# citiususc/veryfasttree

Hardware: AMD Instinct MI355X
Metric: profile-ops/sec (higher is better)
Workload: dtype f32; 1 GPU; c4_1M_x200_nt_tophits; n_seqs=1000000, n_pos=200, active_nodes=750000, top_k=2000

## Files before the change

veryfasttree_amd/csrc/vft_kernels_nj.h:

```cpp
#pragma once
#include "vft_device.h"

#define VFT_WG 256

template <typename REAL>
struct QueryBuf {
    REAL *w;
    uint8_t *code;
    REAL *f;
    uint4 *enc;
    double2 *tab;
};

template <typename REAL>
__device__ __forceinline__ void vft_query_tab(const QueryBuf<REAL> &q, int64_t p, REAL wq, const REAL *f) {
#pragma unroll
    for (int c = 0; c < 5; c++) {
        double2 v = make_double2(0.0, 0.0);
        if (c < 4 && wq > 0) {
            const double wgt = (double) wq;
            const double piece = 1.0 - (double) f[c < 4 ? c : 0];
            v = make_double2(wgt * piece, wgt);
        }
        q.tab[p * 5 + c] = v;
    }
}

template <typename REAL, int NC>
__device__ __forceinline__ void vft_extract_query(const Arena<REAL> &A, int64_t node, const QueryBuf<REAL> &q) {
    const int64_t p = (int64_t) blockIdx.x * blockDim.x + threadIdx.x;
    const int64_t nPosPad = (int64_t) A.d.nChunk * VFT_CHUNK;
    if (p >= nPosPad) return;
    REAL w = 0;
    int code = VFT_NOCODE_;
    REAL f[NC];
#pragma unroll
    for (int k = 0; k < NC; k++) f[k] = 0;
    if (p < A.d.nPos) {
        Col<REAL, NC> c;
        vft_load_col<REAL, NC>(A, node, p, c);
        w = c.w;
        code = c.code;
        if (c.vec) {
#pragma unroll
            for (int k = 0; k < NC; k++) f[k] = c.f[k];
        } else if (NC == 4 && code != VFT_NOCODE_) {
#pragma unroll
            for (int k = 0; k < NC; k++) f[k] = (k == code) ? (REAL) 1 : (REAL) 0;
        }
    }
    q.w[p] = w;
    q.code[p] = (uint8_t) code;
#pragma unroll
    for (int k = 0; k < NC; k++) q.f[p * NC + k] = f[k];
    if (NC == 4) vft_query_tab<REAL>(q, p, w, f);
    if (node < A.d.nSeqs && p < A.d.nChunk) {
        q.enc[p] = A.leafT[vft_leaf_idx(A.d, node >> 6, (int) p, (int) (node & 63))];
    }
}
template <typename REAL, int NC>
__global__ void k_extract_query(Arena<REAL> A, int64_t node, QueryBuf<REAL> q) {
    vft_extract_query<REAL, NC>(A, node, q);
}
#ifdef VFT_NO_PLAIN_COLUMNS
#define VFT_PLAIN_COLUMNS 0
#define VFT_MQ_STRIDE(S) (4 * (S) + 4)
#else
#define VFT_PLAIN_COLUMNS 1
#define VFT_MQ_STRIDE(S) (4 * (S) + 8)
#endif
#ifdef VFT_NO_SEED_CODE_RECORDS
#define VFT_SEED_CODE_RECORDS 0
#else
#define VFT_SEED_CODE_RECORDS 1
#endif
#if defined(VFT_NO_GPR_INDEX_SELECT) || !VFT_SEED_CODE_RECORDS || !VFT_PLAIN_COLUMNS
#define VFT_GPR_INDEX_SELECT 0
#else
#define VFT_GPR_INDEX_SELECT 1
#endif
template <typename REAL>
struct QuerySlot {
    int64_t node;
    QueryBuf<REAL> q;
    REAL *mq;
    int32_t mqIdx, mqS;
    uint32_t *lq;
    int32_t lqIdx, lqS;
};
template <typename REAL, int NC>
__global__ void k_extract_query_batch(Arena<REAL> A, const QuerySlot<REAL> *qs) {
    const QuerySlot<REAL> &sl = qs[blockIdx.y];
    vft_extract_query<REAL, NC>(A, sl.node, sl.q);
    if (VFT_SEED_CODE_RECORDS && NC == 4 && sl.lq) {
        const int64_t p = (int64_t) blockIdx.x * blockDim.x + threadIdx.x;
        if (p < (int64_t) A.d.nChunk * VFT_CHUNK) {
            uint8_t *dst = (uint8_t *) (sl.lq + p);
            dst[sl.lqIdx] = sl.q.code[p];
            if (sl.lqIdx == 0)
                for (int k = sl.lqS; k < 4; k++) dst[k] = VFT_NOCODE_;
        }
    }
    if (NC == 4 && sl.mq) {
        const int64_t p = (int64_t) blockIdx.x * blockDim.x + threadIdx.x;
        if (p < (int64_t) A.d.nChunk * VFT_CHUNK) {
            REAL *dst = sl.mq + p * VFT_MQ_STRIDE(sl.mqS);
#pragma unroll
            for (int k = 0; k < 4; k++) dst[4 * sl.mqIdx + k] = sl.q.f[p * 4 + k];
            dst[4 * sl.mqS + sl.mqIdx] = sl.q.w[p];
            if (VFT_PLAIN_COLUMNS) ((uint8_t *) (dst + 4 * sl.mqS + 4))[sl.mqIdx] = sl.q.code[p];
        }
    }
}

template <typename REAL, int NC>
__global__ void k_outprofile_as_query(Arena<REAL> A, QueryBuf<REAL> q) {
    const int64_t p = (int64_t) blockIdx.x * blockDim.x + threadIdx.x;
    const int64_t nPosPad = (int64_t) A.d.nChunk * VFT_CHUNK;
    if (p >= nPosPad) return;
    const bool in = p < A.d.nPos;
    q.w[p] = in ? A.outW[p] : (REAL) 0;
    q.code[p] = VFT_NOCODE_;
    REAL f[NC];
#pragma unroll
    for (int k = 0; k < NC; k++) {
        f[k] = in ? A.outF[p * NC + k] : (REAL) 0;
        q.f[p * NC + k] = f[k];
    }
    if (NC == 4) vft_query_tab<REAL>(q, p, in ? A.outW[p] : (REAL) 0, f);
}

struct SweepArgs {
    int64_t query;
    int64_t lo, hi;
    int64_t nActive, nDiffAllow;
    double totdiam;
    int32_t queryIsLeaf;
    int32_t force;
    int32_t nLeafWG;
    int32_t pad;
    int64_t leafEnd;
    int64_t heavyLo;
};

template <typename REAL>
struct SweepOut {
    REAL *dist, *weight, *crit;
    REAL *partMin, *partMax;
};

template <typename REAL, int NWAVES>
__device__ __forceinline__ void vft_block_minmax_n(REAL cmin, REAL cmax, REAL *partMin, REAL *partMax, int part) {
    __shared__ REAL smin[NWAVES], smax[NWAVES];
#pragma unroll
    for (int off = 32; off > 0; off >>= 1) {
        const REAL a = __shfl_xor(cmin, off, 64), b = __shfl_xor(cmax, off, 64);
        cmin = a < cmin ? a : cmin;
        cmax = b > cmax ? b : cmax;
    }
    if ((threadIdx.x & 63) == 0) {
        smin[threadIdx.x >> 6] = cmin;
        smax[threadIdx.x >> 6] = cmax;
    }
    __syncthreads();
    if (threadIdx.x == 0) {
#pragma unroll
        for (int w = 1; w < NWAVES; w++) {
            cmin = smin[w] < cmin ? smin[w] : cmin;
            cmax = smax[w] > cmax ? smax[w] : cmax;
        }
        partMin[part] = cmin;
        partMax[part] = cmax;
    }
}
template <typename REAL>
__device__ __forceinline__ void vft_block_minmax(REAL cmin, REAL cmax, REAL *partMin, REAL *partMax, int part) {
    vft_block_minmax_n<REAL, VFT_WG / 64>(cmin, cmax, partMin, partMax, part);
}

enum { MODE_CRIT = 0, MODE_OUTDIST = 1, MODE_CRIT_LEAFQ = 2 };

__device__ __forceinline__ void vft_seq_counts(const uint4 a, const uint4 b, int &nUse, int &nSame) {
    const uint32_t x = a.x & b.x, y = a.y & b.y, z = a.z & b.z, w = a.w & b.w;
    nUse += __popc(x & 0x10101010u) + __popc(y & 0x10101010u) + __popc(z & 0x10101010u) + __popc(w & 0x10101010u);
    nSame += __popc(x & 0x0F0F0F0Fu) + __popc(y & 0x0F0F0F0Fu) + __popc(z & 0x0F0F0F0Fu) + __popc(w & 0x0F0F0F0Fu);
}

#ifndef VFT_SUB
#define VFT_SUB 8
#endif
__device__ __forceinline__ uint32_t vft_query_code(const uint8_t *code, int64_t p0, int b) {
    const uint32_t w = vft_uniform_load<uint32_t>((const uint32_t *) (code + p0 + (b & ~3)));
    return (w >> ((b & 3) * 8)) & 0xFFu;
}
template <typename REAL>
__device__ __forceinline__ uint32_t vft_query_code(const QueryBuf<REAL> &Q, int64_t p0, int b) {
    return vft_query_code(Q.code, p0, b);
}

template <typename REAL, bool QLEAF>
struct IntChunk {
    REAL w[VFT_SUB];
    REAL f[VFT_SUB][QLEAF ? 1 : 4];
};

typedef unsigned int __attribute__((ext_vector_type(4))) vft_u4_t;
typedef unsigned int __attribute__((ext_vector_type(2))) vft_u2_t;
typedef const __attribute__((address_space(4))) vft_u4_t *vft_smask_t;
typedef const __attribute__((address_space(4))) vft_u2_t *vft_soff_t;

#ifdef VFT_ABLATE
#define VFT_ABLATE_BITS(s) ((s).pad)
#else
#define VFT_ABLATE_BITS(s) 0
#endif

template <typename REAL, bool QLEAF>
__device__ __forceinline__ void vft_int_chunk_load(IntChunk<REAL, QLEAF> &r, int c, int sub, const uint4 codes,
                                                   const REAL *wT, vft_smask_t mM, vft_soff_t mO, const REAL *fT,
                                                   const QueryBuf<REAL> &Q, int dbg = 0) {
    const int64_t p0 = (int64_t) c * VFT_CHUNK + sub * VFT_SUB;
    vft_u4_t mk[VFT_SUB];
    vft_u2_t of[VFT_SUB];
#pragma unroll
    for (int b = 0; b < VFT_SUB; b++) {
        mk[b] = mM[p0 + b];
        of[b] = mO[p0 + b];
    }
#pragma unroll
    for (int b = 0; b < VFT_SUB; b++) {
        const unsigned long long mv = ((unsigned long long) mk[b].y << 32) | mk[b].x;
        const unsigned long long mw = ((unsigned long long) mk[b].w << 32) | mk[b].z;
// ... 561 lines not shown
        cur = nxt;
    }
#endif
}

template <typename REAL, int S>
__global__ __launch_bounds__(VFT_WG) void k_sweep_nt_leafq_multi(Arena<REAL> A, MultiLeafQ<REAL, S> M, SweepArgs s) {
    constexpr int SUB = 8;
    REAL cmin[S], cmax[S];
#pragma unroll
    for (int q = 0; q < S; q++) {
        cmin[q] = (REAL) 1e30;
        cmax[q] = (REAL) -1e30;
    }
    const int wg = (int) gridDim.x - 1 - (int) blockIdx.x;
    const int64_t j = s.heavyLo + (int64_t) wg * VFT_WG + threadIdx.x;
    const int lane = (int) (j & 63);
    const int64_t tile = j >> 6;
    bool work = false;
    if (j < s.hi) {
        work = A.parent[j] < 0;
        if (!work) {
#pragma unroll
            for (int q = 0; q < S; q++) {
                M.O[q].dist[j] = (REAL) 1e20;
                M.O[q].crit[j] = (REAL) 1e20;
                M.O[q].weight[j] = 0;
            }
        }
    }
    if (work) {
        const bool targetLeaf = j < A.d.nSeqs;
        REAL dist[S], weight[S];
        if (targetLeaf) {
            int nUse[S], nSame[S];
#pragma unroll
            for (int q = 0; q < S; q++) nUse[q] = nSame[q] = 0;
            for (int c = 0; c < A.d.nChunk; c++) {
                const uint4 t = A.leafT[vft_leaf_idx(A.d, tile, c, lane)];
#pragma unroll
                for (int q = 0; q < S; q++) vft_seq_counts(t, M.Q[q].enc[c], nUse[q], nSame[q]);
            }
#pragma unroll
            for (int q = 0; q < S; q++) {
                const double top = (double) (nUse[q] - nSame[q]);
                weight[q] = (REAL) (double) nUse[q];
                dist[q] = (REAL) (nUse[q] > 0 ? top / (double) nUse[q] : 1.0);
            }
        } else {
            double top[S], denom[S];
#pragma unroll
            for (int q = 0; q < S; q++) top[q] = denom[q] = 0;
            LeafCodes<S> lc;
#if VFT_SEED_CODE_RECORDS
            lc.lq = M.lq;
#else
#pragma unroll
            for (int q = 0; q < S; q++) lc.code[q] = M.Q[q].code;
#endif
            vft_for_column_groups<REAL, SUB>(A, tile, lane, [&](const IntChunkAll<REAL, SUB> &ca, int64_t p0) {
                vft_int_chunk_consume_all<REAL, S, SUB>(ca, p0, lc, top, denom);
            });
#pragma unroll
            for (int q = 0; q < S; q++) {
                weight[q] = (REAL) (denom[q] > 0 ? denom[q] : 0.01);
                dist[q] = (REAL) (denom[q] > 0 ? top[q] / denom[q] : 1.0);
            }
        }
#pragma unroll
        for (int q = 0; q < S; q++) {
            SweepArgs sq = s;
            sq.query = M.query[q];
            vft_sweep_finish<REAL, MODE_CRIT>(A, sq, M.O[q], j, dist[q], weight[q], targetLeaf, cmin[q], cmax[q]);
        }
    }
    vft_block_minmax_multi<REAL, S>(cmin, cmax, M.O, wg);
}

template <int S>
__device__ __forceinline__ void vft_pin_sums(double *top, double *denom) {
#pragma unroll
    for (int q = 0; q < S; q++) asm volatile("" : "+v"(top[q]), "+v"(denom[q]));
}

template <typename REAL, int S>
struct QueryCol {
    REAL w[S];
    typename UVec4<REAL>::type f[S];
    uint32_t codes;
};
template <typename REAL, int S>
__device__ __forceinline__ void vft_query_col_load(QueryCol<REAL, S> &c, const REAL *mq, int64_t p) {
    const REAL *src = mq + p * VFT_MQ_STRIDE(S);
    const typename UVec4<REAL>::type wv = vft_uniform_load4<REAL>(src + 4 * S);
    if (VFT_PLAIN_COLUMNS) c.codes = vft_uniform_load<uint32_t>((const uint32_t *) (src + 4 * S + 4));
#pragma unroll
    for (int q = 0; q < S; q++) {
        c.w[q] = q == 0 ? wv.x : q == 1 ? wv.y : q == 2 ? wv.z : wv.w;
        c.f[q] = vft_uniform_load4<REAL>(src + 4 * q);
    }
}

template <typename REAL, int S, int SUB, bool ISEL = false>
__device__ __forceinline__ void vft_int_chunk_consume_prof(const IntChunkAll<REAL, SUB> &ca, int64_t p0, const REAL *mq, double *top, double *denom) {
    QueryCol<REAL, S> cur, nxt;
    vft_query_col_load<REAL, S>(cur, mq, p0);
#pragma unroll
    for (int b = 0; b < SUB; b++) {
        if (b + 1 < SUB) vft_query_col_load<REAL, S>(nxt, mq, p0 + b + 1);
        __builtin_amdgcn_sched_barrier(0);
#if VFT_SEED_CODE_RECORDS
        const unsigned long long cw = VFT_PLAIN_COLUMNS ? cur.codes : 0;
#endif
        constexpr bool isel = VFT_GPR_INDEX_SELECT && ISEL;
        double fd[S];
#if VFT_GPR_INDEX_SELECT
        if constexpr (ISEL) vft_isel_cvt<S>(fd, ca.f[b], b, cur.codes);
#endif
#pragma unroll
        for (int q = 0; q < S; q++) {
            const REAL ww = cur.w[q] * ca.w[b];
            const double wgt = (double) ww;
            double head = 1.0, lastd = 0;
            REAL last;
            if constexpr (isel) {
                lastd = fd[q];
            } else if (VFT_PLAIN_COLUMNS) {
#if VFT_SEED_CODE_RECORDS
                last = vft_usel_code(ca.f[b], cw, 8 * q);
#else
                const unsigned long long m0 = (cur.codes & (1u << (8 * q))) ? ~0ull : 0ull, m1 = (cur.codes & (2u << (8 * q))) ? ~0ull : 0ull;
                last = vft_usel(vft_usel(ca.f[b].x, ca.f[b].y, m0), vft_usel(ca.f[b].z, ca.f[b].w, m0), m1);
#endif
            }
            if (!VFT_PLAIN_COLUMNS || __builtin_expect((cur.codes & (0x40u << (8 * q))) != 0, 0)) {
                const typename UVec4<REAL>::type pr = cur.f[q] * ca.f[b];
                head = 1.0 - (double) pr.x;
                head -= (double) pr.y;
                head -= (double) pr.z;
                last = pr.w;
                if constexpr (isel) lastd = (double) pr.w;
            }
            if constexpr (!isel) lastd = (double) last;
            const double piece = head - lastd;
            denom[q] += wgt;
            top[q] += wgt * piece;
            if (VFT_PLAIN_COLUMNS) asm volatile("" : "+v"(top[q]), "+v"(denom[q]));
        }
        __builtin_amdgcn_sched_barrier(0);
        if (b + 1 < SUB) cur = nxt;
    }
}

#define VFT_PTILE_M 112
template <int NBT, int S>
__device__ __forceinline__ void vft_leaf_table_chunk_multi(const double2 *row, const uint4 *t, double (*top)[S], double (*denom)[S]) {
    constexpr int GC = NBT * S >= 8 ? 1 : NBT * S >= 4 ? 2 : 4;
#pragma unroll
    for (int g = 0; g < VFT_CHUNK; g += GC) {
        double2 v[NBT][GC][S];
#pragma unroll
        for (int bt = 0; bt < NBT; bt++)
#pragma unroll
            for (int q = 0; q < GC; q++) {
                const int idx = __ffs((int) (vft_byte(t[bt], g + q) | 0x10u)) - 1;
#pragma unroll
                for (int sd = 0; sd < S; sd++) v[bt][q][sd] = row[sd * (VFT_PTILE_M * 5) + (g + q) * 5 + idx];
            }
#pragma unroll
        for (int q = 0; q < GC; q++)
#pragma unroll
            for (int bt = 0; bt < NBT; bt++)
#pragma unroll
                for (int sd = 0; sd < S; sd++) {
                    denom[bt][sd] += v[bt][q][sd].y;
                    top[bt][sd] += v[bt][q][sd].x;
                }
    }
}

template <typename REAL, int NBT, int S>
__device__ __forceinline__ void vft_leaf_table_walk_multi(const Arena<REAL> &A, const MultiLeafQ<REAL, S> &M, double2 *tab, const int64_t *tj,
                                                          double (*top)[S], double (*denom)[S]) {
    const int tid = threadIdx.x;
    const int64_t nPos = A.d.nPos;
    const uint4 *lp[NBT];
#pragma unroll
    for (int bt = 0; bt < NBT; bt++) lp[bt] = A.leafT + vft_leaf_idx(A.d, tj[bt] >> 6, 0, (int) (tj[bt] & 63));
    for (int64_t p0 = 0; p0 < nPos; p0 += VFT_PTILE_M) {
        __syncthreads();
        {
            const int64_t nTab = ((int64_t) A.d.nChunk * VFT_CHUNK - p0) * 5;
#pragma unroll
            for (int sd = 0; sd < S; sd++)
                for (int e = tid; e < VFT_PTILE_M * 5; e += VFT_WG)
                    tab[sd * (VFT_PTILE_M * 5) + e] = e < nTab ? M.Q[sd].tab[p0 * 5 + e] : make_double2(0.0, 0.0);
        }
        __syncthreads();
        const int c0 = (int) (p0 / VFT_CHUNK);
        const int c1 = (int) (((p0 + VFT_PTILE_M < nPos ? p0 + VFT_PTILE_M : nPos) + VFT_CHUNK - 1) / VFT_CHUNK);
        uint4 ta[NBT], tb[NBT];
#pragma unroll
        for (int bt = 0; bt < NBT; bt++) ta[bt] = lp[bt][(int64_t) c0 * VFT_TILE];
        for (int c = c0; c < c1; c += 2) {
            const int cb = c + 1 < c1 ? c + 1 : c, ca = c + 2 < c1 ? c + 2 : c;
#pragma unroll
            for (int bt = 0; bt < NBT; bt++) tb[bt] = lp[bt][(int64_t) cb * VFT_TILE];
            __builtin_amdgcn_sched_barrier(0);
            vft_leaf_table_chunk_multi<NBT, S>(tab + (int64_t) (c - c0) * VFT_CHUNK * 5, ta, top, denom);
#pragma unroll
            for (int bt = 0; bt < NBT; bt++) ta[bt] = lp[bt][(int64_t) ca * VFT_TILE];
            __builtin_amdgcn_sched_barrier(0);
            if (c + 1 < c1) vft_leaf_table_chunk_multi<NBT, S>(tab + (int64_t) (c + 1 - c0) * VFT_CHUNK * 5, tb, top, denom);
        }
    }
}

template <typename REAL, int S>
__device__ __forceinline__ void vft_leaf_table_wg_multi(const Arena<REAL> &A, const MultiLeafQ<REAL, S> &M, const SweepArgs &s, int64_t base,
                                                        REAL *cmin, REAL *cmax) {
    constexpr int NB = VFT_LEAF_SPAN / VFT_WG, NW = VFT_WG / 64, NBT = 2;
    __shared__ double2 tab[S * VFT_PTILE_M * 5];
    __shared__ unsigned short list[VFT_LEAF_SPAN];
    __shared__ int segCnt[NB * NW];
    const int tid = threadIdx.x, wave = tid >> 6;
    unsigned long long bal[NB];
#pragma unroll
    for (int r = 0; r < NB; r++) {
        const int64_t j = base + r * VFT_WG + tid;
        bool active = false;
        if (j < s.leafEnd) {
            active = A.parent[j] < 0;
            if (!active) {
#pragma unroll
                for (int q = 0; q < S; q++) {
                    M.O[q].dist[j] = (REAL) 1e20;
                    M.O[q].crit[j] = (REAL) 1e20;
                    M.O[q].weight[j] = 0;
                }
            }
        }
        bal[r] = __ballot(active);
        if ((tid & 63) == 0) segCnt[r * NW + wave] = __popcll(bal[r]);
    }
    __syncthreads();
    int nAct = 0, off[NB];
#pragma unroll
    for (int seg = 0; seg < NB * NW; seg++) {
#pragma unroll
        for (int r = 0; r < NB; r++)
            if (seg == r * NW + wave) off[r] = nAct;
        nAct += segCnt[seg];
    }
#pragma unroll
    for (int r = 0; r < NB; r++) {
        const int rank = (int) __builtin_amdgcn_mbcnt_hi((unsigned int) (bal[r] >> 32), __builtin_amdgcn_mbcnt_lo((unsigned int) bal[r], 0u));
        if ((bal[r] >> (tid & 63)) & 1ull) list[off[r] + rank] = (unsigned short) (r * VFT_WG + tid);
    }
    __syncthreads();
    for (int r0 = 0; r0 < nAct; r0 += NBT * VFT_WG) {
        int64_t tj[NBT];
        double top[NBT][S], denom[NBT][S];
#pragma unroll
        for (int bt = 0; bt < NBT; bt++) {
            const int idx = r0 + bt * VFT_WG + tid;
            tj[bt] = base + list[idx < nAct ? idx : 0];
#pragma unroll
            for (int q = 0; q < S; q++) top[bt][q] = denom[bt][q] = 0;
        }
        if (nAct - r0 <= VFT_WG) vft_leaf_table_walk_multi<REAL, 1, S>(A, M, tab, tj, top, denom);
        else vft_leaf_table_walk_multi<REAL, NBT, S>(A, M, tab, tj, top, denom);
#pragma unroll
        for (int bt = 0; bt < NBT; bt++) {
            if (r0 + bt * VFT_WG + tid < nAct) {
#pragma unroll
                for (int q = 0; q < S; q++) {
                    const REAL weight = (REAL) (denom[bt][q] > 0 ? denom[bt][q] : 0.01);
                    const REAL dist = (REAL) (denom[bt][q] > 0 ? top[bt][q] / denom[bt][q] : 1.0);
                    SweepArgs sq = s;
                    sq.query = M.query[q];
                    vft_sweep_finish<REAL, MODE_CRIT>(A, sq, M.O[q], tj[bt], dist, weight, false, cmin[q], cmax[q]);
                }
            }
        }
    }
}

#define VFT_KARG __attribute__((address_space(4)))
template <typename T>
__device__ __forceinline__ const VFT_KARG T *vft_kernarg(size_t off) {
    const VFT_KARG char *p = (const VFT_KARG char *) __builtin_amdgcn_kernarg_segment_ptr() + off;
    asm volatile("" : "+s"(p));
    return (const VFT_KARG T *) p;
}
template <typename REAL>
__device__ __forceinline__ SweepOut<REAL> vft_karg_out(const VFT_KARG SweepOut<REAL> *p) {
    typedef __attribute__((address_space(1))) REAL *gp_t;
    SweepOut<REAL> o;
    o.dist = (REAL *) (gp_t) p->dist;
    o.weight = (REAL *) (gp_t) p->weight;
    o.crit = (REAL *) (gp_t) p->crit;
    o.partMin = (REAL *) (gp_t) p->partMin;
    o.partMax = (REAL *) (gp_t) p->partMax;
    return o;
}
template <typename REAL, int S>
__device__ __forceinline__ void vft_karg_sentinels(const VFT_KARG MultiLeafQ<REAL, S> *M, int64_t j) {
#pragma unroll
    for (int q = 0; q < S; q++) {
        const SweepOut<REAL> O = vft_karg_out<REAL>(&M->O[q]);
        O.dist[j] = (REAL) 1e20;
        O.crit[j] = (REAL) 1e20;
        O.weight[j] = 0;
    }
}
template <typename REAL, int S>
__device__ __forceinline__ void vft_block_minmax_karg(REAL *cmin, REAL *cmax, const VFT_KARG MultiLeafQ<REAL, S> *M, int part,
                                                      REAL (*smin)[VFT_WG / 64], REAL (*smax)[VFT_WG / 64]) {
    constexpr int NW = VFT_WG / 64;
#pragma unroll
    for (int q = 0; q < S; q++) {
#pragma unroll
        for (int off = 32; off > 0; off >>= 1) {
            const REAL a = __shfl_xor(cmin[q], off, 64), b = __shfl_xor(cmax[q], off, 64);
            cmin[q] = a < cmin[q] ? a : cmin[q];
            cmax[q] = b > cmax[q] ? b : cmax[q];
        }
        if ((threadIdx.x & 63) == 0) {
            smin[q][threadIdx.x >> 6] = cmin[q];
            smax[q][threadIdx.x >> 6] = cmax[q];
        }
    }
    __syncthreads();
    if (threadIdx.x < S) {
        const int q = threadIdx.x;
        REAL lo = smin[q][0], hi = smax[q][0];
#pragma unroll
        for (int w = 1; w < NW; w++) {
            lo = smin[q][w] < lo ? smin[q][w] : lo;
            hi = smax[q][w] > hi ? smax[q][w] : hi;
        }
        const SweepOut<REAL> O = vft_karg_out<REAL>(&M->O[q]);
        O.partMin[part] = lo;
        O.partMax[part] = hi;
    }
}

template <typename REAL, int S>
__global__ __launch_bounds__(VFT_WG, sizeof(REAL) == 4 ? 3 : 2) void k_sweep_nt_profq_multi(Arena<REAL> A, MultiLeafQ<REAL, S> M, SweepArgs s) {
    constexpr int SUB = 8;
    __shared__ REAL smin[S][VFT_WG / 64], smax[S][VFT_WG / 64];
    const int nT = s.nLeafWG, nHeavy = (int) gridDim.x - nT, blk = (int) blockIdx.x;
    REAL cmin[S], cmax[S];
#pragma unroll
    for (int q = 0; q < S; q++) {
        cmin[q] = (REAL) 1e30;
        cmax[q] = (REAL) -1e30;
    }
    if (blk >= nHeavy) {
        const int span = blk - nHeavy;
        vft_leaf_table_wg_multi<REAL, S>(A, M, s, s.lo + (int64_t) span * VFT_LEAF_SPAN, cmin, cmax);
        vft_block_minmax_multi<REAL, S>(cmin, cmax, M.O, span);
        return;
    }
    const int wg = nHeavy - 1 - blk;
    const int64_t j = s.heavyLo + (int64_t) wg * VFT_WG + threadIdx.x;
    const int lane = (int) (j & 63);
    const int64_t tile = j >> 6;
    constexpr size_t offM = (sizeof(Arena<REAL>) + alignof(MultiLeafQ<REAL, S>) - 1) / alignof(MultiLeafQ<REAL, S>) * alignof(MultiLeafQ<REAL, S>);
    const VFT_KARG MultiLeafQ<REAL, S> *M0 = vft_kernarg<MultiLeafQ<REAL, S>>(offM);
    bool work = false;
    if (j < s.hi && !(nT && j < s.leafEnd)) {
        work = A.parent[j] < 0;
        if (!work) vft_karg_sentinels<REAL, S>(M0, j);
    }
    double top[S], denom[S];
#pragma unroll
    for (int q = 0; q < S; q++) top[q] = denom[q] = 0;
    const VFT_KARG MultiLeafQ<REAL, S> *M1 = vft_kernarg<MultiLeafQ<REAL, S>>(offM);
    if (work) {
        const REAL *mq = M1->mq;
        vft_for_column_groups<REAL, SUB>(A, tile, lane, [&](const IntChunkAll<REAL, SUB> &ca, int64_t p0) {
            vft_int_chunk_consume_prof<REAL, S, SUB, sizeof(REAL) == 4>(ca, p0, mq, top, denom);
            vft_pin_sums<S>(top, denom);
        });
    }
    const VFT_KARG MultiLeafQ<REAL, S> *Mk = vft_kernarg<MultiLeafQ<REAL, S>>(offM);
    if (work) {
#pragma unroll
        for (int q = 0; q < S; q++) {
            const REAL weight = (REAL) (denom[q] > 0 ? denom[q] : 0.01);
            const REAL dist = (REAL) (denom[q] > 0 ? top[q] / denom[q] : 1.0);
            SweepArgs sq = s;
            sq.query = Mk->query[q];
            vft_sweep_finish<REAL, MODE_CRIT>(A, sq, vft_karg_out<REAL>(&Mk->O[q]), j, dist, weight, false, cmin[q], cmax[q]);
        }
    }
    vft_block_minmax_karg<REAL, S>(cmin, cmax, vft_kernarg<MultiLeafQ<REAL, S>>(offM), nT + wg, smin, smax);
}

template <typename REAL, int SL, int SP>
struct MixedQ {
    MultiLeafQ<REAL, SL> L;
    MultiLeafQ<REAL, SP> P;
};
template <typename REAL, int SL, int SP>
struct MixedArgs {
    Arena<REAL> A;
    SweepArgs s;
    int32_t nInt, nLeafHeavy;
    MixedQ<REAL, SL, SP> M;
};
template <typename REAL, int SL, int SP>
__global__ __launch_bounds__(VFT_WG, sizeof(REAL) == 4 ? 3 : 2) void k_sweep_nt_mixed_multi(MixedArgs<REAL, SL, SP> a) {
    typedef MixedArgs<REAL, SL, SP> Args;
    constexpr int SUB = 8, NW = VFT_WG / 64;
    constexpr size_t offL = offsetof(Args, M) + offsetof(decltype(Args::M), L), offP = offsetof(Args, M) + offsetof(decltype(Args::M), P);
    __shared__ REAL smin[SL + SP][NW], smax[SL + SP][NW];
    const Arena<REAL> &A = a.A;
    const SweepArgs &s = a.s;
    const int blk = (int) blockIdx.x, nInt = a.nInt, nLH = a.nLeafHeavy, nT = s.nLeafWG;
    REAL cminP[SP], cmaxP[SP], cminL[SL], cmaxL[SL];
#pragma unroll
    for (int q = 0; q < SP; q++) {
        cminP[q] = (REAL) 1e30;
        cmaxP[q] = (REAL) -1e30;
    }
#pragma unroll
    for (int q = 0; q < SL; q++) {
        cminL[q] = (REAL) 1e30;
        cmaxL[q] = (REAL) -1e30;
    }
    if (blk >= nInt + nLH) {
        const int span = blk - nInt - nLH;
        const VFT_KARG MultiLeafQ<REAL, SP> *Pk = vft_kernarg<MultiLeafQ<REAL, SP>>(offP);
        MultiLeafQ<REAL, SP> M;
#pragma unroll
        for (int q = 0; q < SP; q++) {
            M.Q[q].w = Pk->Q[q].w;
            M.Q[q].code = Pk->Q[q].code;
            M.Q[q].f = Pk->Q[q].f;
            M.Q[q].enc = Pk->Q[q].enc;
            M.Q[q].tab = Pk->Q[q].tab;
            M.O[q] = vft_karg_out<REAL>(&Pk->O[q]);
            M.query[q] = Pk->query[q];
        }
        M.mq = Pk->mq;
        vft_leaf_table_wg_multi<REAL, SP>(A, M, s, s.lo + (int64_t) span * VFT_LEAF_SPAN, cminP, cmaxP);
        vft_block_minmax_karg<REAL, SP>(cminP, cmaxP, vft_kernarg<MultiLeafQ<REAL, SP>>(offP), span, smin, smax);
        return;
    }
    if (blk >= nInt) {
        const int wg = nLH - 1 - (blk - nInt);
        const int64_t j = s.lo + (int64_t) wg * VFT_WG + threadIdx.x;
        const VFT_KARG MultiLeafQ<REAL, SL> *Lk = vft_kernarg<MultiLeafQ<REAL, SL>>(offL);
        bool work = false;
        if (j < s.leafEnd) {
            work = A.parent[j] < 0;
            if (!work) vft_karg_sentinels<REAL, SL>(Lk, j);
        }
        if (work) {
            const uint4 *enc[SL];
            int nUse[SL], nSame[SL];
#pragma unroll
            for (int q = 0; q < SL; q++) {
                enc[q] = Lk->Q[q].enc;
                nUse[q] = nSame[q] = 0;
            }
            const int lane = (int) (j & 63);
            const int64_t tile = j >> 6;
            for (int c = 0; c < A.d.nChunk; c++) {
                const uint4 t = A.leafT[vft_leaf_idx(A.d, tile, c, lane)];
#pragma unroll
                for (int q = 0; q < SL; q++) vft_seq_counts(t, enc[q][c], nUse[q], nSame[q]);
            }
#pragma unroll
            for (int q = 0; q < SL; q++) {
                const double top = (double) (nUse[q] - nSame[q]);
                const REAL weight = (REAL) (double) nUse[q];
                const REAL dist = (REAL) (nUse[q] > 0 ? top / (double) nUse[q] : 1.0);
                SweepArgs sq = s;
                sq.query = Lk->query[q];
                vft_sweep_finish<REAL, MODE_CRIT>(A, sq, vft_karg_out<REAL>(&Lk->O[q]), j, dist, weight, true, cminL[q], cmaxL[q]);
            }
        }
        vft_block_minmax_karg<REAL, SL>(cminL, cmaxL, vft_kernarg<MultiLeafQ<REAL, SL>>(offL), wg, smin, smax);
        return;
    }
    const int wg = nInt - 1 - blk;
    const int64_t j = s.heavyLo + (int64_t) wg * VFT_WG + threadIdx.x;
    const int lane = (int) (j & 63);
    const int64_t tile = j >> 6;
    const VFT_KARG MixedQ<REAL, SL, SP> *M0 = vft_kernarg<MixedQ<REAL, SL, SP>>(offsetof(Args, M));
    bool work = false;
    if (j < s.hi && j >= s.leafEnd) {
        work = A.parent[j] < 0;
        if (!work) {
            vft_karg_sentinels<REAL, SP>(&M0->P, j);
            vft_karg_sentinels<REAL, SL>(&M0->L, j);
        }
    }
    double topP[SP], denomP[SP], topL[SL], denomL[SL];
#pragma unroll
    for (int q = 0; q < SP; q++) topP[q] = denomP[q] = 0;
#pragma unroll
    for (int q = 0; q < SL; q++) topL[q] = denomL[q] = 0;
    const VFT_KARG MixedQ<REAL, SL, SP> *M1 = vft_kernarg<MixedQ<REAL, SL, SP>>(offsetof(Args, M));
    if (work) {
        const REAL *mq = M1->P.mq;
        LeafCodes<SL> lc;
#if VFT_SEED_CODE_RECORDS
        lc.lq = M1->L.lq;
#else
#pragma unroll
        for (int q = 0; q < SL; q++) lc.code[q] = M1->L.Q[q].code;
#endif
        vft_for_column_groups<REAL, SUB>(A, tile, lane, [&](const IntChunkAll<REAL, SUB> &ca, int64_t p0) {
            vft_int_chunk_consume_prof<REAL, SP, SUB, sizeof(REAL) == 4>(ca, p0, mq, topP, denomP);
            vft_pin_sums<SP>(topP, denomP);
            __builtin_amdgcn_sched_barrier(0);
            vft_int_chunk_consume_all<REAL, SL, SUB, true, sizeof(REAL) == 4>(ca, p0, lc, topL, denomL);
            vft_pin_sums<SL>(topL, denomL);
            __builtin_amdgcn_sched_barrier(0);
        });
    }
    const VFT_KARG MixedQ<REAL, SL, SP> *Mk = vft_kernarg<MixedQ<REAL, SL, SP>>(offsetof(Args, M));
    if (work) {
#pragma unroll
        for (int q = 0; q < SP; q++) {
            const REAL weight = (REAL) (denomP[q] > 0 ? denomP[q] : 0.01);
            const REAL dist = (REAL) (denomP[q] > 0 ? topP[q] / denomP[q] : 1.0);
            SweepArgs sq = s;
            sq.query = Mk->P.query[q];
            vft_sweep_finish<REAL, MODE_CRIT>(A, sq, vft_karg_out<REAL>(&Mk->P.O[q]), j, dist, weight, false, cminP[q], cmaxP[q]);
        }
#pragma unroll
        for (int q = 0; q < SL; q++) {
            const REAL weight = (REAL) (denomL[q] > 0 ? denomL[q] : 0.01);
            const REAL dist = (REAL) (denomL[q] > 0 ? topL[q] / denomL[q] : 1.0);
            SweepArgs sq = s;
            sq.query = Mk->L.query[q];
            vft_sweep_finish<REAL, MODE_CRIT>(A, sq, vft_karg_out<REAL>(&Mk->L.O[q]), j, dist, weight, false, cminL[q], cmaxL[q]);
        }
    }
    vft_block_minmax_karg<REAL, SP>(cminP, cmaxP, vft_kernarg<MultiLeafQ<REAL, SP>>(offP), nT + wg, smin, smax);
    vft_block_minmax_karg<REAL, SL>(cminL, cmaxL, vft_kernarg<MultiLeafQ<REAL, SL>>(offL), nLH + wg, smin + SP, smax + SP);
}

template <typename REAL, int NC>
__device__ __forceinline__ void vft_pair_generic(const Arena<REAL> &A, int64_t i, int64_t j, bool jIsOut, REAL &dist,
                                                 REAL &weight) {
    const int64_t nPos = A.d.nPos;
    if (!jIsOut && i < A.d.nSeqs && j < A.d.nSeqs) {
        double top = 0;
        int64_t nUse = 0;
        int nDiff = 0;
        const int li = (int) (i & 63), lj = (int) (j & 63);
        for (int c = 0; c < A.d.nChunk; c++) {
            const uint4 a = A.leafT[vft_leaf_idx(A.d, i >> 6, c, li)];
            const uint4 b = A.leafT[vft_leaf_idx(A.d, j >> 6, c, lj)];
            for (int t = 0; t < VFT_CHUNK; t++) {
                if ((int64_t) c * VFT_CHUNK + t >= nPos) break;
                const int ca = vft_decode<NC>(vft_byte(a, t)), cb = vft_decode<NC>(vft_byte(b, t));
                if (ca != VFT_NOCODE_ && cb != VFT_NOCODE_) {
                    nUse++;
                    if (A.dmDist) top += (double) A.dmDist[ca * NC + cb];
                    else if (ca != cb) nDiff++;
                }
            }
        }
        if (!A.dmDist) top = (double) nDiff;
        weight = (REAL) (double) nUse;
        dist = (REAL) (nUse > 0 ? top / (double) nUse : 1.0);
        return;
    }
    double top = 0, denom = 0;
    for (int64_t p = 0; p < nPos; p++) {
        Col<REAL, NC> c1, c2;
        vft_load_col<REAL, NC>(A, i, p, c1);
        if (jIsOut) {
            c2.w = A.outW[p];
            c2.code = VFT_NOCODE_;
            c2.vec = c2.w > 0;
#pragma unroll
            for (int k = 0; k < NC; k++) c2.f[k] = A.outF[p * NC + k];
        } else {
            vft_load_col<REAL, NC>(A, j, p, c2);
        }
        if (c1.w > 0 && c2.w > 0) {
            const REAL ww = c1.w * c2.w;
            const double wgt = (double) ww;
            denom += wgt;
            const double piece = vft_piece<REAL, NC>(A, c1, c2, (jIsOut && A.outCD) ? A.outCD + p * NC : nullptr);
            top += wgt * piece;
        }
    }
    weight = (REAL) (denom > 0 ? denom : 0.01);
    dist = (REAL) (denom > 0 ? top / denom : 1.0);
}

template <typename REAL, int NC>
__device__ __forceinline__ void vft_pair_load(const Arena<REAL> &A, int64_t i, int64_t j, bool jIsOut, int64_t p,
                                              Col<REAL, NC> &c1, Col<REAL, NC> &c2, bool iRow, bool jRow) {
    if (iRow) vft_load_row<REAL, NC>(A, i, p, c1);
    else vft_load_col<REAL, NC>(A, i, p, c1);
    if (jIsOut) {
        c2.w = A.outW[p];
        c2.code = VFT_NOCODE_;
        c2.vec = c2.w > 0;
#pragma unroll
        for (int k = 0; k < NC; k++) c2.f[k] = A.outF[p * NC + k];
    } else if (jRow) {
        vft_load_row<REAL, NC>(A, j, p, c2);
    } else {
        vft_load_col<REAL, NC>(A, j, p, c2);
    }
}
template <typename REAL>
__device__ __forceinline__ bool vft_is_row(const Arena<REAL> &A, int64_t node) {
#ifdef VFT_AB_NO_ROWS
    return false;
#endif
    return node >= A.d.nSeqs && A.mlIs != nullptr && A.mlIs[node - A.d.nSeqs] != 0;
}
template <typename REAL, int NC>
__device__ __forceinline__ void vft_pair_wave(const Arena<REAL> &A, int64_t i, int64_t j, bool jIsOut, double *sW,
                                              double *sT, REAL &dist, REAL &weight) {
    const int lane = threadIdx.x & 63;
    const int64_t nPos = A.d.nPos;
    const bool leaves = !jIsOut && i < A.d.nSeqs && j < A.d.nSeqs;
    if (leaves && !A.dmDist && NC == 4) {
        int nUse = 0, nSame = 0;
        for (int c = lane; c < A.d.nChunk; c += 64)
            vft_seq_counts(A.leafT[vft_leaf_idx(A.d, i >> 6, c, (int) (i & 63))],
                           A.leafT[vft_leaf_idx(A.d, j >> 6, c, (int) (j & 63))], nUse, nSame);
#pragma unroll
        for (int off = 32; off > 0; off >>= 1) {
            nUse += __shfl_xor(nUse, off, 64);
            nSame += __shfl_xor(nSame, off, 64);
        }
        weight = (REAL) (double) nUse;
        dist = (REAL) (nUse > 0 ? (double) (nUse - nSame) / (double) nUse : 1.0);
        return;
    }
    const bool iRow = vft_is_row<REAL>(A, i), jRow = !jIsOut && vft_is_row<REAL>(A, j);
    for (int64_t p = lane; p < nPos; p += 128) {
        const int64_t pb = p + 64;
        const bool hasB = pb < nPos;
        Col<REAL, NC> a1, a2, b1, b2;
        vft_pair_load<REAL, NC>(A, i, j, jIsOut, p, a1, a2, iRow, jRow);
        if (hasB) vft_pair_load<REAL, NC>(A, i, j, jIsOut, pb, b1, b2, iRow, jRow);
        vft_pair_addends<REAL, NC>(A, leaves, jIsOut, p, a1, a2, sW, sT);
        if (hasB) vft_pair_addends<REAL, NC>(A, leaves, jIsOut, pb, b1, b2, sW, sT);
    }
    __builtin_amdgcn_fence(__ATOMIC_RELEASE, "wavefront");
    __builtin_amdgcn_wave_barrier();
    __builtin_amdgcn_fence(__ATOMIC_ACQUIRE, "wavefront");
    double acc = 0;
    if (lane < 2) {
        const double *src = lane == 0 ? sT : sW;
        int64_t p = 0;
        for (; p + 8 <= nPos; p += 8) {
            double v[8];
#pragma unroll
            for (int u = 0; u < 8; u++) v[u] = src[p + u];
#pragma unroll
            for (int u = 0; u < 8; u++) acc += v[u];
        }
        for (; p < nPos; p++) acc += src[p];
    }
// ... 976 lines not shown
```

Before: 15.23 billion profile-ops/s.

## Share per-column 1-f pieces across seeds via GPR-indexed multiply

Adds a shared-pieces path for f32 that computes the four per-column pieces (1 - f_c) once and selects the right one per seed with s_set_gpr_idx indexed v_mul_f64 in inline asm. The profile and leaf seeds then reuse these pieces instead of each recomputing the dot-product head. Rare mixed-code columns fall back to the full computation. This cuts double-precision ALU work per column. The cost is pinned physical registers v96-v103 and M0 usage, which can constrain register allocation, and the path assumes exactly four seeds.

```diff
diff --git a/veryfasttree_amd/csrc/vft_kernels_nj.h b/veryfasttree_amd/csrc/vft_kernels_nj.h
--- a/veryfasttree_amd/csrc/vft_kernels_nj.h
+++ b/veryfasttree_amd/csrc/vft_kernels_nj.h
@@ -78,6 +78,11 @@
 #define VFT_GPR_INDEX_SELECT 0
 #else
 #define VFT_GPR_INDEX_SELECT 1
+#endif
+#if defined(VFT_NO_SHARED_PIECES) || !VFT_GPR_INDEX_SELECT
+#define VFT_SHARED_PIECES 0
+#else
+#define VFT_SHARED_PIECES 1
 #endif
 template <typename REAL>
 struct QuerySlot {
@@ -945,6 +950,92 @@
     }
 }
 
+#if VFT_SHARED_PIECES
+#define VFT_PIECE_V0 96
+#pragma clang diagnostic push
+#pragma clang diagnostic ignored "-Winline-asm"
+template <int S>
+__device__ __forceinline__ void vft_ipiece_mul(double *prod, double P0, double P1, double P2, double P3, const double *w, uint32_t cw) {
+    static_assert(S == 4, "a full seed group of vft_sweep_batch (for two seeds the four pieces cost more than they save)");
+    static_assert(VFT_PIECE_V0 == 96, "the register names below");
+    uint32_t t0, t1, t2, t3;
+    asm("s_lshl_b32 %4, %16, 1\n\t"
+        "s_and_b32 %4, %4, 6\n\t"
+        "s_bfe_u32 %5, %16, 0x30007\n\t"
+        "s_bfe_u32 %6, %16, 0x3000f\n\t"
+        "s_bfe_u32 %7, %16, 0x30017\n\t"
+        "s_set_gpr_idx_on %4, gpr_idx(SRC0)\n\t"
+        "v_mul_f64 %0, v[96:97], %12\n\t"
+        "s_set_gpr_idx_idx %5\n\t"
+        "v_mul_f64 %1, v[96:97], %13\n\t"
+        "s_set_gpr_idx_idx %6\n\t"
+        "v_mul_f64 %2, v[96:97], %14\n\t"
+        "s_set_gpr_idx_idx %7\n\t"
+        "v_mul_f64 %3, v[96:97], %15\n\t"
+        "s_set_gpr_idx_off"
+        : "=&v"(prod[0]), "=&v"(prod[1]), "=&v"(prod[2]), "=&v"(prod[3]), "=&s"(t0), "=&s"(t1), "=&s"(t2), "=&s"(t3)
+        : "{v[96:97]}"(P0), "{v[98:99]}"(P1), "{v[100:101]}"(P2), "{v[102:103]}"(P3), "v"(w[0]), "v"(w[1]), "v"(w[2]), "v"(w[3]), "s"(cw)
+        : "scc", "m0");
+}
+#pragma clang diagnostic pop
+
+template <int SL, int SP, int SUB>
+__device__ __forceinline__ void vft_int_chunk_consume_shared(const IntChunkAll<float, SUB> &ca, int64_t p0, const float *mq, const uint32_t *lq,
+                                                             double *topP, double *denomP, double *topL, double *denomL) {
+    static_assert(SUB == 8, "a group's codes are one 8-dword load");
+    typedef unsigned long long __attribute__((ext_vector_type(4))) vft_ul4_t;
+    vft_ul4_t rec;
+    if constexpr (SL > 0) rec = *(const __attribute__((address_space(4))) vft_ul4_t *) (lq + p0);
+    QueryCol<float, SP> cur, nxt;
+    vft_query_col_load<float, SP>(cur, mq, p0);
+#pragma unroll
+    for (int b = 0; b < SUB; b++) {
+        if (b + 1 < SUB) vft_query_col_load<float, SP>(nxt, mq, p0 + b + 1);
+        __builtin_amdgcn_sched_barrier(0);
+        const double P0 = 1.0 - (double) ca.f[b].x, P1 = 1.0 - (double) ca.f[b].y, P2 = 1.0 - (double) ca.f[b].z, P3 = 1.0 - (double) ca.f[b].w;
+        {
+            double wgt[SP], prod[SP];
+#pragma unroll
+            for (int q = 0; q < SP; q++) {
+                const float ww = cur.w[q] * ca.w[b];
+                wgt[q] = (double) ww;
+            }
+            vft_ipiece_mul<SP>(prod, P0, P1, P2, P3, wgt, cur.codes);
+#pragma unroll
+            for (int q = 0; q < SP; q++) {
+                if (__builtin_expect((cur.codes & (0x40u << (8 * q))) != 0, 0)) {
+                    const UVec4<float>::type pr = cur.f[q] * ca.f[b];
+                    double head = 1.0 - (double) pr.x;
+                    head -= (double) pr.y;
+                    head -= (double) pr.z;
+                    prod[q] = wgt[q] * (head - (double) pr.w);
+                }
+                denomP[q] += wgt[q];
+                topP[q] += prod[q];
+                asm volatile("" : "+v"(topP[q]), "+v"(denomP[q]));
+            }
+        }
+        if constexpr (SL > 0) {
+            const unsigned long long w2 = b < 2 ? rec.x : b < 4 ? rec.y : b < 6 ? rec.z : rec.w;
+            const uint32_t cw = (uint32_t) (w2 >> (32 * (b & 1)));
+            const double wd = (double) ca.w[b];
+            const double w4[4] = {wd, wd, wd, wd};
+            double prod[SL > 0 ? SL : 1];
+            vft_ipiece_mul<SL>(prod, P0, P1, P2, P3, w4, cw);
+#pragma unroll
+            for (int q = 0; q < SL; q++) {
+                if (__builtin_expect((cw & (0x40u << (8 * q))) != 0, 0)) continue;
+                denomL[q] += wd;
+                topL[q] += prod[q];
+                asm volatile("" : "+v"(topL[q]), "+v"(denomL[q]));
+            }
+        }
+        __builtin_amdgcn_sched_barrier(0);
+        if (b + 1 < SUB) cur = nxt;
+    }
+}
+#endif
+
 #define VFT_PTILE_M 112
 template <int NBT, int S>
 __device__ __forceinline__ void vft_leaf_table_chunk_multi(const double2 *row, const uint4 *t, double (*top)[S], double (*denom)[S]) {
@@ -1174,7 +1265,11 @@
     if (work) {
         const REAL *mq = M1->mq;
         vft_for_column_groups<REAL, SUB>(A, tile, lane, [&](const IntChunkAll<REAL, SUB> &ca, int64_t p0) {
-            vft_int_chunk_consume_prof<REAL, S, SUB, sizeof(REAL) == 4>(ca, p0, mq, top, denom);
+#if VFT_SHARED_PIECES
+            if constexpr (sizeof(REAL) == 4 && S == 4) vft_int_chunk_consume_shared<0, S, SUB>(ca, p0, mq, nullptr, top, denom, nullptr, nullptr);
+            else
+#endif
+                vft_int_chunk_consume_prof<REAL, S, SUB, sizeof(REAL) == 4>(ca, p0, mq, top, denom);
             vft_pin_sums<S>(top, denom);
         });
     }
@@ -1309,6 +1404,15 @@
         for (int q = 0; q < SL; q++) lc.code[q] = M1->L.Q[q].code;
 #endif
         vft_for_column_groups<REAL, SUB>(A, tile, lane, [&](const IntChunkAll<REAL, SUB> &ca, int64_t p0) {
+#if VFT_SHARED_PIECES
+            if constexpr (sizeof(REAL) == 4) {
+                vft_int_chunk_consume_shared<SL, SP, SUB>(ca, p0, mq, lc.lq, topP, denomP, topL, denomL);
+                vft_pin_sums<SP>(topP, denomP);
+                vft_pin_sums<SL>(topL, denomL);
+                __builtin_amdgcn_sched_barrier(0);
+                return;
+            }
+#endif
             vft_int_chunk_consume_prof<REAL, SP, SUB, sizeof(REAL) == 4>(ca, p0, mq, topP, denomP);
             vft_pin_sums<SP>(topP, denomP);
             __builtin_amdgcn_sched_barrier(0);
```

Result: faster. 15.49 billion profile-ops/s (median of 6 runs) (+1.7%).
